# Alfieriek/Python-Temporal-AME-SVI

Measured on AMD Instinct MI355X. Metric: dyad-timestep ELBO updates/sec at n=1024,T=128,d=16; 1/2/4/8-GPU scaling, higher is better.
Workload: dtype f32

## Files before the change

python-temporal-ame-svi_amd/ame_amd/csrc/ame_sweep3.hip:

```cpp
#include "ame_common.h"
#include "ame_wave.h"
#include "ame_sweep_dev.h"

using namespace ame;

namespace {
__device__ __forceinline__ Mat2 inv2s_fast(Mat2 m) {
    const double det = m.a * m.d - m.b * m.c;
    double r = __builtin_amdgcn_rcp(det);
    r = fma(r, fma(-det, r, 1.0), r);
    r = fma(r, fma(-det, r, 1.0), r);
    const double o = 0.5 * (-m.b * r - m.c * r);
    return {m.d * r, o, o, m.a * r};
}
}

#ifdef AME_STAMPS
#define S3_I0 256
__device__ unsigned long long g_s3_stamps[8 * 16 * 16];
__device__ unsigned long long g_s3_prog[256 * 5];
__device__ unsigned int g_s3_hwid[8];
#define S3W(w) (w)
#define STAMP3(slot)                                                                           \
    do {                                                                                       \
// ... 101 lines not shown
    const int n = dm.n, TL = dm.T_local, Tt = dm.T_total;
    const int b = blockIdx.x;
    const int tl = (TL % 8 == 0) ? ((b & 7) * (TL >> 3) + (b >> 3)) : b;
    const int tg = dm.t_begin + tl;
    const int tid = threadIdx.x, lane = tid & 63, wave = __builtin_amdgcn_readfirstlane(tid >> 6);
    const int hl = tid - 64, hw = wave - 1;
    const int hj = (hl + kNH - kGOFF) % kNH;
    constexpr bool is_naive = VAR == AME_NAIVE, is_bad = VAR == AME_BAD;
    const int ns = (n + kNH - 1) / kNH;
    const int NY = (n * 8 + 1023) / 1024;
    const int KDMA = NY + NC + 2;

    extern __shared__ __attribute__((aligned(16))) char smem[];
    using LY = Lay<R>;
    const int YS = LY::ys(n);
    double* Kbuf = (double*)(smem + LY::oK);
    constexpr int KS = LY::KS, KSZ = LY::KSZ;
    constexpr int MCP = LY::MCP;
    double* arQ = (double*)(smem + LY::oAR);
    double* arP = arQ + D * MCP;
    double* rec = (double*)(smem + LY::oRec);
    double* mu64 = (double*)(smem + LY::oMu64);
    float* mu32 = (float*)(smem + LY::oMu32);
    double* g64 = (double*)(smem + LY::oG);
    double* jn64 = (double*)(smem + LY::oJn);
    double* vbuf = (double*)(smem + LY::oV);
    double* red = (double*)(smem + LY::oRed);
    float* gp = (float*)(smem + LY::oGP);
    float* yst = (float*)(smem + LY::oYst);
    float* muL = (float*)(smem + LY::oMuL);
    double* pdl = (double*)(smem + LY::oPd);
    double* pcdl = (double*)(smem + LY::oPc);
    double* ssq = (double*)(smem + LY::oSq);
    uint32_t* flags = (uint32_t*)(smem + LY::oFlag);
    uint32_t* kcnt = flags;
    uint32_t* gcnt = flags + 2;
    float2* yring = (float2*)(smem + LY::oYr);
    float* cring = (float*)(smem + LY::oCr);
    float* xring = (float*)(smem + LY::oXr);
    float* rring = (float*)(smem + LY::oRr);
    uint64_t* pring = (uint64_t*)(smem + LY::oPr);
    float* cst = (float*)(smem + LY::oCs);
    float2* mlds = (float2*)(smem + LY::oML(n));

    const double r00 = a.rinv[0], r01 = a.rinv[1], r10 = a.rinv[2], r11 = a.rinv[3];
    const float r00f = (float)r00, r01f = (float)r01, r10f = (float)r10, r11f = (float)r11;
    const Mat2 Rm = inv2s(m2(r00, r01, r10, r11));
    const float lr = a.lr, om = a.one_minus_lr;
    const float* xo = a.x_old + (size_t)tl * n * D;
    float* xn = a.x_new + (size_t)tl * n * D;
    float* cvs = a.cov + (size_t)tl * n * DD;
    float* cvw = (a.cov_new != nullptr ? a.cov_new : a.cov) + (size_t)tl * n * DD;
    const int nys = ame_ystride(n);
    const float* ysl = a.Yt + (size_t)tl * n * nys * 2;
    const bool back_rd = (a.wait_epoch != 0u) && (tl == TL - 1) && (a.back_in != nullptr);
    const float* xr = (tg < Tt - 1) ? ((tl < TL - 1) ? a.x_old + (size_t)(tl + 1) * n * D
                                                     : (back_rd ? a.back_in : a.next_old))
                                    : nullptr;
    const double* QiPhi = a.consts + 3 * (size_t)DD;
    bool dead = false;

    auto gran_src = [&](int node) -> const uint64_t* {
        return (tl == 0) ? a.halo_in + (size_t)node * D : a.hand + ((size_t)(tl - 1) * n + node) * D;
    };
    auto gran_finish = [&](int node, uint64_t v, float* dst) {
        if (tg == 0) {
            if (lane < D) dst[lane] = 0.f;
            return;
        }
        bool ok = (lane >= D) || (uint32_t)(v >> 32) == a.epoch;
        if (!__all(ok) && !dead) {
            const bool cross = tl == 0 && !(a.flags & AME_SWEEP_FLAG_PREV_GROUP);
            AmeSpin w(a.status, cross, lane == 0, hw == 0 ? AME_ST_HALO_US : 0);
            const uint64_t* src = gran_src(node);
            while (true) {
                bool stale = false;
                if (lane < D) {
                    v = cross ? gran_load_system(src + lane) : gran_load_agent(src + lane);
                    ok = (uint32_t)(v >> 32) == a.epoch;
                    stale = (uint32_t)(v >> 32) > a.epoch;
                }
                const bool st_hit = __any(stale);
                if (__all(ok) && !st_hit) break;
                const int r = st_hit ? 3 : w.poll();
                if (r != 0) {
                    const uint64_t bad = __ballot(!ok);
                    const int fl = bad ? (int)__builtin_ctzll(bad) : 0;
                    const uint32_t obs = (uint32_t)(__shfl(v, fl) >> 32);
                    if (lane == 0 && r >= 2)
                        ame_fail(a.status, (r == 3) ? AME_STATUS_STALE_EPOCH
                                                    : (cross ? AME_STATUS_HALO_TIMEOUT : AME_STATUS_SPIN_TIMEOUT),
                                 cross ? AME_WAIT_GRAN_HALO : AME_WAIT_GRAN_LOCAL, tg, (uint32_t)node, obs,
                                 a.epoch, w.waited(), a.epoch);
                    if (lane == 0)
                        __hip_atomic_fetch_or(gcnt, AME_LDS_DEAD, __ATOMIC_RELAXED, __HIP_MEMORY_SCOPE_WORKGROUP);
                    dead = true;
                    break;
                }
                __builtin_amdgcn_s_sleep(2);
            }
            w.end();
        }
        if (lane < D) dst[lane] = __uint_as_float((uint32_t)v);
    };

    auto dma_y = [&](int row) {
        const int rw = (row < n) ? row : 0;
        const char* base = (const char*)(ysl + (size_t)rw * nys * 2);
        const uint32_t dst = lds_off(yring + (size_t)(row & 3) * YS);
        for (int q = 0; q < NY; ++q) {
            int off = (q * 64 + lane) * 16;
            if (off >= n * 8) off = 0;
            dma16(base + off, dst + q * 1024);
        }
    };
    auto dma_cov = [&](int node) {
        const int cn = (node >= 0 && node < n) ? node : 0;
        const char* base = (const char*)(cvs + (size_t)cn * DD);
        const uint32_t dst = lds_off(cring + (size_t)(node & 3) * LY::cs);
#pragma unroll
        for (int q = 0; q < NC; ++q) {
            int off = (q * 64 + lane) * 16;
            if (off >= DD * 4) off = 0;
            dma16(base + off, dst + q * 1024);
        }
    };
    auto dma_x = [&](int node) {
        const int xnn = (node < n) ? node : 0;
        dma4(xo + (size_t)xnn * D + (lane < D ? lane : 0), lds_off(xring + (node & 7) * 64));
    };
    auto dma_r = [&](int node) {
        const float* src = (xr != nullptr && node < n) ? xr + (size_t)node * D : xo;
        if (back_rd) dma4_sys(src + (lane < D ? lane : 0), lds_off(rring + (node & 3) * 64));
        else dma4(src + (lane < D ? lane : 0), lds_off(rring + (node & 3) * 64));
    };

    auto flush_cov = [&](int node) {
        const float4* src = (const float4*)(cst + (size_t)((node + 1) & 1) * LY::cs);
        float4* dst = (float4*)(cvw + (size_t)node * DD);
#pragma unroll
        for (int q = 0; q < NC; ++q) {
            const int e = q * 64 + lane;
            if (e * 4 < DD) dst[e] = src[e];
        }
    };

#ifdef AME_STAMPS
    if (tl == TL / 2 && lane == 0) {
        unsigned int hwid;
        asm volatile("s_getreg_b32 %0, hwreg(HW_REG_HW_ID)" : "=s"(hwid));
        g_s3_hwid[wave] = hwid;
    }
#endif
    if (a.wait_epoch != 0u) {
        if (tid == 0) ame_wait_prev_done(a, tl, TL, tg, back_rd, n * D, dead);
        __syncthreads();
    }
    {
        double* piv = vbuf;
        double* K = Kbuf;
        const double pp = r00, ss = r11, qq = 0.5 * (r01 + r10);
        double* colsum = vbuf;
        float* x0 = (float*)(vbuf + M2);
        p0_gram_mfma<R, kNT / 64>(xo, n, D, K, KS, colsum, x0);
        if (tid < M2) {
            const int kq = 2 + (tid >= R ? tid - R : tid + R);
            const double v = (double)x0[tid];
            ssq[2 + tid] = fma(v, v, K[kq * KS + kq]);
        }
        __syncthreads();
        for (int e = tid; e < NLT; e += kNT) {
            int k, m;
            tri_decode3(e, k, m);
            double v;
            if (k < 2) {
                v = ((k == 0 && m == 0) ? pp : (k == 1 && m == 1) ? ss : qq) * (double)(n - 1);
            } else {
                const bool ku = (k - 2) < R;
                if (m < 2) {
                    const int ck = k - 2, kc = (ck < R) ? R + ck : ck - R;
                    v = (ku ? (m == 0 ? pp : qq) : (m == 0 ? qq : ss)) * colsum[kc];
                } else {
                    const bool mu_ = (m - 2) < R;
                    v = ((ku && mu_) ? pp : ((!ku && !mu_) ? ss : qq)) * K[k * KS + m];
                }
            }
            v += pconst_entry(a.consts, D, k, m, tg, Tt);
            K[k * KS + m] = v;
            K[m * KS + k] = v;
        }
        __syncthreads();
        for (int pv = 0; pv < D; ++pv) {
            if (tid < D) piv[tid] = K[pv * KS + tid];
            __syncthreads();
            const double rinv = 1.0 / piv[pv];
            for (int e = tid; e < NLT; e += kNT) {
                int k, m;
                tri_decode3(e, k, m);
                double v;
                if (k == pv && m == pv) v = -rinv;
                else if (k == pv) v = piv[m] * rinv;
                else if (m == pv) v = piv[k] * rinv;
                else v = K[k * KS + m] - (piv[k] * piv[m]) * rinv;
                K[k * KS + m] = v;
                K[m * KS + k] = v;
            }
            __syncthreads();
        }
        for (int e = tid; e < KSZ; e += kNT) K[e] = -K[e];
        __syncthreads();
    }
    for (int e = tid; e < 2 * D * MCP; e += kNT) {
        const int mat = e / (D * MCP), rc = e - mat * D * MCP, rr = rc / MCP, cc = rc - rr * MCP;
        arQ[e] = (cc < D) ? QiPhi[(size_t)mat * DD + rr * D + cc] : 0.0;
    }
    for (int e = tid; e < 3 * 64; e += kNT) muL[e] = 0.f;
    if (tid < D) pcdl[tid] = pconst_entry(a.consts, D, tid, tid, tg, Tt);
    constexpr int RS = LY::RS;
    for (int e = tid; e < 2 * D * RS; e += kNT) rec[e] = 0.0;
    for (int e = tid; e < 2 * D; e += kNT) {
        mu64[e] = 0.0;
        mu32[e] = 0.f;
    }
    if (tid < 16) yst[tid] = 0.f;
    if (tid < 4) flags[tid] = 0u;
    float mreg[NSREG][M2];
    if (wave >= 1) {
#pragma unroll
        for (int s = 0; s < NSREG; ++s) {
            const int j = hj + kNH * s;
            const bool ok = s < ns && j < n;
#pragma unroll
            for (int c = 0; c < M2; ++c) mreg[s][c] = ok ? xo[(size_t)j * D + 2 + c] : 0.f;
        }
        for (int s = NSREG; s < ns; ++s) {
            const int j = hj + kNH * s;
            const bool ok = j < n;
            for (int c2 = 0; c2 < MP; ++c2) {
                float2 v = make_float2(0.f, 0.f);
                if (ok) {
                    v.x = xo[(size_t)j * D + 2 + 2 * c2];
                    if (2 * c2 + 1 < M2) v.y = xo[(size_t)j * D + 3 + 2 * c2];
                }
                mlds[((s - NSREG) * MP + c2) * kNH + hl] = v;
            }
        }
        for (int e = hl; e < 2 * n; e += kNH) {
            const int rw = e / n, j = e - rw * n;
            yring[(size_t)rw * YS + j] = (rw < n) ? *(const float2*)(ysl + ((size_t)rw * nys + j) * 2)
                                                    : make_float2(0.f, 0.f);
        }
    }
    if (wave == 7) {
        for (int q = 0; q < 5; ++q) dma_x(q);
        for (int q = 0; q < 4; ++q) dma_r(q);
        asm volatile("s_waitcnt vmcnt(0)" ::: "memory");
    }
    __syncthreads();

    auto gemv = [&](int m, const float2* ysrc, int i) {
        float acc[D];
#pragma unroll
        for (int c = 0; c < D; ++c) acc[c] = 0.f;
        float2 yv[NSREG];
#pragma unroll
        for (int s = 0; s < NSREG; ++s) {
            const int j = hj + kNH * s;
            const float2 y = ysrc[j];
            yv[s] = (j < n) ? y : make_float2(0.f, 0.f);
        }
#pragma unroll
        for (int s = 0; s < NSREG; ++s) {
            if (s < ns) {
                const int j = hj + kNH * s;
                const bool ex = (j >= m - 2) && (j <= m);
                const float z0 = ex ? 0.f : r00f * yv[s].x + r01f * yv[s].y;
                const float z1 = ex ? 0.f : r10f * yv[s].x + r11f * yv[s].y;
                acc[0] += z0;
                acc[1] += z1;
#pragma unroll
                for (int c = 0; c < R; ++c) {
                    acc[2 + c] = fmaf(z0, mreg[s][R + c], acc[2 + c]);
                    acc[2 + R + c] = fmaf(z1, mreg[s][c], acc[2 + R + c]);
                }
            }
        }
        for (int s = NSREG; s < ns; ++s) {
            const int j = hj + kNH * s;
            float2 y = ysrc[j];
            if (j >= n) y = make_float2(0.f, 0.f);
            const bool ex = (j >= m - 2) && (j <= m);
            const float z0 = ex ? 0.f : r00f * y.x + r01f * y.y;
            const float z1 = ex ? 0.f : r10f * y.x + r11f * y.y;
            acc[0] += z0;
            acc[1] += z1;
            const float2* ml = mlds + (size_t)(s - NSREG) * MP * kNH + hl;
#pragma unroll
            for (int c2 = 0; c2 < MP; ++c2) {
                const float2 t = ml[c2 * kNH];
                const int c = 2 * c2;
                if (c < R) acc[2 + R + c] = fmaf(z1, t.x, acc[2 + R + c]);
                else acc[2 + (c - R)] = fmaf(z0, t.x, acc[2 + (c - R)]);
                if (c + 1 < M2) {
                    if (c + 1 < R) acc[2 + R + c + 1] = fmaf(z1, t.y, acc[2 + R + c + 1]);
                    else acc[2 + (c + 1 - R)] = fmaf(z0, t.y, acc[2 + (c + 1 - R)]);
                }
            }
        }
        STAMP3(7);
        int idx;
        const float v = wave_reduce_scatter<D>(acc, lane, idx);
        STAMP3(8);
        if (idx < D) gp[((m & 1) * 7 + hw) * D + idx] = v;
        const int jm1 = m - 1, jm2 = m - 2;
        if (jm1 >= 0 && ((jm1 + kGOFF) % kNH) == hl) {
            const float2 y = ysrc[jm1];
            yst[(m & 3) * 4 + 0] = y.x;
            yst[(m & 3) * 4 + 1] = y.y;
        }
        if (jm2 >= 0 && ((jm2 + kGOFF) % kNH) == hl) {
            const float2 y = ysrc[jm2];
            yst[(m & 3) * 4 + 2] = y.x;
            yst[(m & 3) * 4 + 3] = y.y;
        }
    };
    auto hf1 = [&](int m) {
        const int q = hl;
        const int k = q / NP, p = q - k * NP;
        const int kc = (k < D) ? k : 0;
        const float* ml = muL + hw * 64;
        const float* mr = rring + (m & 3) * 64;
        const double* aq = arQ + kc * MCP + p * MC;
        const double* ap = arP + kc * MCP + p * MC;
        double av[MC], bv[MC];
        float lv[MC], rv[MC], gv[7];
#pragma unroll
        for (int mm = 0; mm < MC; ++mm) {
            av[mm] = aq[mm];
            bv[mm] = ap[mm];
            lv[mm] = ml[p * MC + mm];
            rv[mm] = mr[p * MC + mm];
        }
#pragma unroll
        for (int w = 0; w < 7; ++w) gv[w] = gp[((m & 1) * 7 + w) * D + kc];
        const float mv2 = jcol_load<R>(mu32 + ((m - 2) & 1) * D, kc);
        const float ys0 = yst[(m & 3) * 4 + 2], ys1 = yst[(m & 3) * 4 + 3];
        __builtin_amdgcn_sched_barrier(0);
        double accL = 0.0, accR = 0.0;
#pragma unroll
        for (int mm = 0; mm < MC; ++mm) {
            accL = fma(av[mm], (double)lv[mm], accL);
            accR = fma(bv[mm], (double)rv[mm], accR);
        }
        double acc = accL + ((tg < Tt - 1) ? accR : 0.0);
        acc = dpp_add_xor1(acc);
        if constexpr (NP == 4) acc = dpp_add_mirror4(acc);
        double g = 0.0;
#pragma unroll
        for (int w = 0; w < 7; ++w) g += (double)gv[w];
        g += acc;
        if (m >= 2) {
            double j0, j1;
            jcol_sel<R>(mv2, true, kc, j0, j1);
            const double y0 = (double)ys0, y1 = (double)ys1;
            const double z0 = r00 * y0 + r01 * y1, z1 = r10 * y0 + r11 * y1;
            g = fma(j0, z0, fma(j1, z1, g));
        }
        if (k < D && p == 0) g64[(m & 1) * D + k] = g;
    };
    auto jn_fill = [&](int node) {
        if (lane < M2) {
            const float* xm = xring + (node & 7) * 64;
            jn64[(node & 1) * 2 * D + lane] = (node < n) ? (double)xm[2 + lane] : 0.0;
        }
    };

    if (wave >= 1) {
        gemv(0, yring, -1);
        gemv(1, yring + YS, -1);
        if (hw <= 2) {
            uint64_t g0 = 0;
            if (tg > 0 && lane < D)
                g0 = (tl == 0) ? gran_load_system(gran_src(0) + lane) : gran_load_agent(gran_src(0) + lane);
            gran_finish(0, g0, muL + hw * 64);
        }
        if (hw == 3) jn_fill(1);
    }
    __syncthreads();
    if (wave >= 1 && hw <= 2) hf1(0);
    __syncthreads();
    if (wave == 7) {
        for (int q = 2; q <= 4; ++q) dma_y(q);
        for (int q = 0; q <= 1; ++q) dma_cov(q);
        asm volatile("s_waitcnt vmcnt(0)" ::: "memory");
    }
    if (wave == 6 && lane < D) {
        uint64_t g1 = 0;
        if (tg > 0 && n > 1)
            g1 = (tl == 0) ? gran_load_system(gran_src(1) + lane) : gran_load_agent(gran_src(1) + lane);
        pring[(size_t)1 * 128 + lane] = g1;
    }
    __syncthreads();

    if (wave == 0) {
        __builtin_amdgcn_s_setprio(3);
        dead = __any(dead) || (*(volatile uint32_t*)gcnt & AME_LDS_DEAD) != 0u;
        const int k = lane;
        const bool kl = k < D;
        const int kc = kl ? k : 0;
        double brow[D];
#pragma unroll
        for (int c = 0; c < D; ++c) brow[c] = kl ? Kbuf[(size_t)k * KS + c] : 0.0;
        double v = 0, yv0 = 0, yv1 = 0, vA = 0, nq0 = 0, nq1 = 0;
        auto prep = [&](int node) {
            const double* jx = jn64 + ((node + 1) & 1) * 2 * D;
            if (!kl) return;
            const double* gg = g64 + (node & 1) * D;
            const bool ex1 = node + 1 < n;
            double s0 = 0, t0 = 0, s1 = ex1 ? brow[0] : 0.0, t1 = 0, s2 = ex1 ? brow[1] : 0.0, t2 = 0;
#pragma unroll
            for (int c = 0; c < D; c += 2) {
                s0 = fma(brow[c], gg[c], s0);
                t0 = fma(brow[c + 1], gg[c + 1], t0);
            }
#pragma unroll
            for (int c = 0; c < R; c += 2) {
                s1 = fma(brow[2 + c], jx[R + c], s1);
                s2 = fma(brow[2 + R + c], jx[c], s2);
                if (c + 1 < R) {
                    t1 = fma(brow[3 + c], jx[R + c + 1], t1);
                    t2 = fma(brow[3 + R + c], jx[c + 1], t2);
                }
            }
            v = s0 + t0;
            yv0 = s1 + t1;
            yv1 = s2 + t2;
            vA = brow[0] * gg[0] + brow[1] * gg[1];
            const double xj = jx[(k >= 2 && k < 2 + R) ? k - 2 + R : ((k >= 2 + R && k < D) ? k - 2 - R : 0)];
            nq0 = (k == 0) ? (ex1 ? 1.0 : 0.0) : ((k >= 2 && k < 2 + R) ? xj : 0.0);
            nq1 = (k == 1) ? (ex1 ? 1.0 : 0.0) : ((k >= 2 + R && k < D) ? xj : 0.0);
        };
        prep(0);
        double Wp0 = 0, Wp1 = 0, Xp0 = 0, Xp1 = 0, Lp0 = 0, Lp1 = 0, Gp0 = 0, Gp1 = 0;
        Mat2 Mip = m2(0, 0, 0, 0), Sip = m2(0, 0, 0, 0);
        for (int i = 0; i < n; ++i) {
            PROG3();
            STAMP3(0);
            const int par = i & 1, ppar = (i + 1) & 1;
            const bool has_prev = i > 0;
            const float* mup = mu32 + ppar * D;
            const double* mupd = mu64 + ppar * D;
            const double msk = kl ? 1.0 : 0.0;
            const double g = msk * g64[par * D + kc];
#if AME_S3_MOLD_EARLY
            const float mold_pf = xring[(i & 7) * 64 + kc];
#endif
            double J0, J1;
            jcol<R>(mup, has_prev && kl, kc, J0, J1);
            double kj0 = 0, kj1 = 0;
            if (has_prev) {
                double s0a = brow[0], s0b = 0, s1a = brow[1], s1b = 0;
#pragma unroll
                for (int c = 0; c < R; c += 2) {
                    s0a = fma(brow[2 + c], mupd[2 + R + c], s0a);
                    s1a = fma(brow[2 + R + c], mupd[2 + c], s1a);
                    if (c + 1 < R) {
                        s0b = fma(brow[3 + c], mupd[3 + R + c], s0b);
                        s1b = fma(brow[3 + R + c], mupd[3 + c], s1b);
                    }
                }
                kj0 = s0a + s0b;
                kj1 = s1a + s1b;
            }
            STAMP3(1);
            constexpr bool pack = is_naive;
            constexpr int NV = is_bad ? 40 : (pack ? 32 : 34);
            constexpr int IE = pack ? 11 : 12, IJY = IE + 2, INY = IJY + 4;
            constexpr int IB = INY + (pack ? 3 : 4), IF1 = IB + 4, IF2 = IF1 + 4;
            double pr[NV];
            pr[0] = Wp0 * J0; pr[1] = Wp0 * J1; pr[2] = Wp1 * J0; pr[3] = Wp1 * J1;
            pr[4] = Xp0 * J0; pr[5] = Xp0 * J1; pr[6] = Xp1 * J0; pr[7] = Xp1 * J1;
            if constexpr (!pack) {
                pr[8] = J0 * kj0; pr[9] = J0 * kj1; pr[10] = J1 * kj0; pr[11] = J1 * kj1;
            } else {
                pr[8] = J0 * kj0; pr[9] = 0.5 * (J0 * kj1 + J1 * kj0); pr[10] = J1 * kj1;
            }
            pr[IE] = J0 * v; pr[IE + 1] = J1 * v;
            pr[IJY] = J0 * yv0; pr[IJY + 1] = J0 * yv1; pr[IJY + 2] = J1 * yv0; pr[IJY + 3] = J1 * yv1;
            if constexpr (!pack) {
                pr[INY] = nq0 * yv0; pr[INY + 1] = nq0 * yv1; pr[INY + 2] = nq1 * yv0; pr[INY + 3] = nq1 * yv1;
            } else {
                pr[INY] = nq0 * yv0; pr[INY + 1] = 0.5 * (nq0 * yv1 + nq1 * yv0); pr[INY + 2] = nq1 * yv1;
            }
            pr[IB] = Wp0 * g; pr[IB + 1] = Wp1 * g; pr[IB + 2] = Xp0 * g; pr[IB + 3] = Xp1 * g;
            pr[IF1] = Wp0 * nq0; pr[IF1 + 1] = Wp0 * nq1; pr[IF1 + 2] = Wp1 * nq0; pr[IF1 + 3] = Wp1 * nq1;
            pr[IF2] = Xp0 * nq0; pr[IF2 + 1] = Xp0 * nq1; pr[IF2 + 2] = Xp1 * nq0; pr[IF2 + 3] = Xp1 * nq1;
            if constexpr (is_bad) {
                const double gA = (k < 2) ? g : 0.0;
                pr[34] = J0 * vA; pr[35] = J1 * vA;
                pr[36] = Wp0 * gA; pr[37] = Wp1 * gA; pr[38] = Xp0 * gA; pr[39] = Xp1 * gA;
            }
            {
                int idx;
                const double sv = wave_reduce_scatter<NV>(pr, lane, idx);
                if (idx < NV) red[idx] = sv;
            }
            wave_lds_sync3();
            double o[NV];
#pragma unroll
            for (int q = 0; q < NV; ++q) o[q] = red[q];
            const Mat2 a1 = m2(o[0], o[1], o[2], o[3]);
            const Mat2 a2 = m2(o[4], o[5], o[6], o[7]);
            const Mat2 cc = !pack ? m2(o[8], o[9], o[10], o[11]) : m2(o[8], o[9], o[9], o[10]);
            const V2 e = {o[IE], o[IE + 1]};
            const Mat2 jy = m2(o[IJY], o[IJY + 1], o[IJY + 2], o[IJY + 3]);
            const Mat2 ny = !pack ? m2(o[INY], o[INY + 1], o[INY + 2], o[INY + 3])
                                   : m2(o[INY], o[INY + 1], o[INY + 1], o[INY + 2]);
            STAMP3(2);
            STAMP3(3);
            const V2 b1 = {o[IB], o[IB + 1]}, b2 = {o[IB + 2], o[IB + 3]};
            const Mat2 f1 = m2(o[IF1], o[IF1 + 1], o[IF1 + 2], o[IF1 + 3]);
            const Mat2 f2 = m2(o[IF2], o[IF2 + 1], o[IF2 + 2], o[IF2 + 3]);
            double y0 = 0, y1 = 0;
            if (has_prev) { y0 = (double)yst[(i & 3) * 4 + 0]; y1 = (double)yst[(i & 3) * 4 + 1]; }
            const double zp0 = r00 * y0 + r01 * y1, zp1 = r10 * y0 + r11 * y1;
            const Mat2 JW = add(sub(cc, quad(a1, Mip, a1)), quad(a2, Sip, a2));
            const Mat2 Mm = add(Rm, sym(JW));
            const Mat2 Mi = has_prev ? inv2s_fast(Mm) : m2(0, 0, 0, 0);
            const V2 t1 = mtv(a1, mv(Mip, b1)), t2 = mtv(a2, mv(Sip, b2));
            const V2 Ju = {e.x - t1.x + t2.x, e.y - t1.y + t2.y};
            const V2 cvec = mv(Mi, V2{y0 - Ju.x, y1 - Ju.y});
            const Mat2 wn = add(sub(jy, quad(a1, Mip, f1)), quad(a2, Sip, f2));
            const Mat2 JnK = add(sub(ny, quad(f1, Mip, f1)), quad(f2, Sip, f2));
            const Mat2 JnX = sub(JnK, quad(wn, Mi, wn));
            const Mat2 Si = inv2s_fast(sub(Rm, sym(JnX)));
            const double W0 = kj0 - (Lp0 * a1.a + Lp1 * a1.c) + (Gp0 * a2.a + Gp1 * a2.c);
            const double W1 = kj1 - (Lp0 * a1.b + Lp1 * a1.d) + (Gp0 * a2.b + Gp1 * a2.d);
            const double u = v - (Lp0 * b1.x + Lp1 * b1.y) + (Gp0 * b2.x + Gp1 * b2.y);
            const double kn0 = yv0 - (Lp0 * f1.a + Lp1 * f1.c) + (Gp0 * f2.a + Gp1 * f2.c);
            const double kn1 = yv1 - (Lp0 * f1.b + Lp1 * f1.d) + (Gp0 * f2.b + Gp1 * f2.d);
            double mus;
            if constexpr (!is_bad) {
                mus = u + W0 * cvec.x + W1 * cvec.y;
            } else {
                const V2 eA = {o[34], o[35]};
                const V2 b1A = {o[36], o[37]}, b2A = {o[38], o[39]};
                const double uA = vA - (Lp0 * b1A.x + Lp1 * b1A.y) + (Gp0 * b2A.x + Gp1 * b2A.y);
// ... 319 lines not shown
```

python-temporal-ame-svi_amd/ame_amd/csrc/ame_sweep_dev.h:

```cpp
#pragma once
#include "ame_common.h"
#include "ame_wave.h"

namespace ame {

__device__ __forceinline__ void lds_barrier3() {
    asm volatile("s_waitcnt lgkmcnt(0)" ::: "memory");
    __builtin_amdgcn_s_barrier();
    asm volatile("" ::: "memory");
}
__device__ __forceinline__ void wave_lds_sync3() {
    asm volatile("s_waitcnt lgkmcnt(0)" ::: "memory");
    __builtin_amdgcn_wave_barrier();
    asm volatile("" ::: "memory");
}
__device__ __forceinline__ void lds_signal_add(uint32_t* f, uint32_t v) {
    asm volatile("s_waitcnt lgkmcnt(0)" ::: "memory");
    __hip_atomic_fetch_add(f, v, __ATOMIC_RELAXED, __HIP_MEMORY_SCOPE_WORKGROUP);
}
__device__ __forceinline__ void lds_signal_set(uint32_t* f, uint32_t v) {
    asm volatile("s_waitcnt lgkmcnt(0)" ::: "memory");
    __hip_atomic_store(f, v, __ATOMIC_RELAXED, __HIP_MEMORY_SCOPE_WORKGROUP);
}
#define AME_LDS_DEAD 0x40000000u
static __device__ __attribute__((noinline)) uint32_t lds_wait_slow(uint32_t* f, uint32_t target, uint32_t* status,
                                                                   int slice, uint32_t node, uint32_t epoch) {
    const bool ld = (threadIdx.x & 63) == 0;
    AmeSpin w(status, false, ld);
    uint32_t v;
    while ((v = __hip_atomic_load(f, __ATOMIC_RELAXED, __HIP_MEMORY_SCOPE_WORKGROUP)) < target) {
        __builtin_amdgcn_s_sleep(8);
        const int r = w.poll();
        if (r == 0) continue;
        if (r == 2 && ld)
            ame_fail(status, AME_STATUS_LDS_TIMEOUT, AME_WAIT_LDS, slice, node, v, target, w.waited(), epoch);
        v |= AME_LDS_DEAD;
        break;
    }
    w.end();
    return v;
}
__device__ __forceinline__ void lds_wait_ge(uint32_t* f, uint32_t target, uint32_t* status, bool& dead,
                                            int slice = 0, uint32_t node = AME_NODE_NONE,
                                            uint32_t epoch = 0) {
    uint32_t v = __hip_atomic_load(f, __ATOMIC_RELAXED, __HIP_MEMORY_SCOPE_WORKGROUP);
    if (!dead && v < target) v = lds_wait_slow(f, target, status, slice, node, epoch);
    dead = dead || (v & AME_LDS_DEAD) != 0u;
    asm volatile("" ::: "memory");
}

__device__ __forceinline__ void ame_wait_prev_done(const ame_sweep_args& a, int t, int TL, int tg,
                                                   bool back_rd, int nd, bool& dead, bool account = true) {
    const int qn = (t + 1 < TL || (a.flags & AME_SWEEP_FLAG_NEXT_GROUP)) ? 2 : 1;
    for (int q = 0; q <= qn && !dead; ++q) {
        const bool back = q == qn;
        if (back && !back_rd) break;
        const uint32_t* w = back ? (const uint32_t*)(a.back_in + AME_BACK_DONE_OFFSET(nd)) : a.done + t + q;
        const int site = back ? AME_WAIT_BACK : (q == 0 ? AME_WAIT_DONE_SELF : AME_WAIT_DONE_RIGHT);
        auto load = [&]() -> uint32_t {
            return back ? __hip_atomic_load(const_cast<uint32_t*>(w), __ATOMIC_RELAXED, __HIP_MEMORY_SCOPE_SYSTEM)
                        : __hip_atomic_load(const_cast<uint32_t*>(w), __ATOMIC_RELAXED, __HIP_MEMORY_SCOPE_AGENT);
        };
        uint32_t dv = load();
        if (dv == a.wait_epoch) continue;
        AmeSpin sp(a.status, back, true, (back && account) ? AME_ST_BACK_US : 0);
        while (true) {
            if (dv > a.wait_epoch) {
                ame_fail(a.status, AME_STATUS_STALE_EPOCH, site, tg, AME_NODE_NONE, dv, a.wait_epoch,
                         sp.waited(), a.epoch);
                dead = true;
                break;
            }
            if (dv == a.wait_epoch) break;
            const int r = sp.poll();
            if (r != 0) {
                if (r == 2)
                    ame_fail(a.status, back ? AME_STATUS_HALO_TIMEOUT : AME_STATUS_SPIN_TIMEOUT, site, tg,
                             AME_NODE_NONE, dv, a.wait_epoch, sp.waited(), a.epoch);
                dead = true;
                break;
            }
            __builtin_amdgcn_s_sleep(8);
            dv = load();
        }
        sp.end();
    }
    if (back_rd) __builtin_amdgcn_fence(__ATOMIC_ACQUIRE, "");
    __builtin_amdgcn_fence(__ATOMIC_ACQUIRE, "agent");
    asm volatile("s_waitcnt vmcnt(0)" ::: "memory");
}

typedef double ame_p0d4 __attribute__((ext_vector_type(4)));
template <int R, int NW>
__device__ __forceinline__ void p0_gram_mfma(const float* xo, int n, int D, double* gram, int ks,
                                             double* colsum, float* x0) {
    constexpr int M2 = 2 * R, NT = (M2 + 15) / 16, NTL = NT * (NT + 1) / 2;
    const int tid = threadIdx.x, lane = tid & 63, w = tid >> 6;
    const int ci = lane & 15, ck = lane >> 4;
    ame_p0d4 acc[NTL];
#pragma unroll
    for (int t = 0; t < NTL; ++t) acc[t] = ame_p0d4{0.0, 0.0, 0.0, 0.0};
    double cs[NT];
#pragma unroll
    for (int I = 0; I < NT; ++I) cs[I] = 0.0;
    const int nch = (n + 3) / 4;
    constexpr int U = 4;
    for (int c0 = w; c0 < nch; c0 += NW * U) {
        float xv[U][NT];
#pragma unroll
        for (int u = 0; u < U; ++u) {
            const int j = 4 * (c0 + NW * u) + ck;
#pragma unroll
            for (int I = 0; I < NT; ++I) {
                const int col = 16 * I + ci;
                const bool ok = j >= 1 && j < n && col < M2;
                xv[u][I] = ok ? xo[(size_t)j * D + 2 + col] : 0.f;
            }
        }
#pragma unroll
        for (int u = 0; u < U; ++u) {
            double xd[NT];
#pragma unroll
            for (int I = 0; I < NT; ++I) {
                xd[I] = (double)xv[u][I];
                cs[I] += xd[I];
            }
#pragma unroll
            for (int I = 0; I < NT; ++I)
#pragma unroll
                for (int J = 0; J <= I; ++J) {
                    const int t = I * (I + 1) / 2 + J;
                    acc[t] = __builtin_amdgcn_mfma_f64_16x16x4f64(xd[I], xd[J], acc[t], 0, 0, 0);
                }
        }
    }
#pragma unroll
    for (int I = 0; I < NT; ++I) {
        const double s1 = cs[I] + __shfl_xor(cs[I], 16);
        cs[I] = s1 + __shfl_xor(s1, 32);
    }
    auto kk = [](int a) { return 2 + (a >= R ? a - R : a + R); };
    for (int ww = 0; ww < NW; ++ww) {
        if (w == ww) {
#pragma unroll
            for (int I = 0; I < NT; ++I)
#pragma unroll
                for (int J = 0; J <= I; ++J) {
                    const int t = I * (I + 1) / 2 + J;
#pragma unroll
                    for (int v = 0; v < 4; ++v) {
                        const int a = 16 * I + ck + 4 * v, b = 16 * J + ci;
                        if (a >= M2 || b >= M2) continue;
                        double* p = gram + kk(a) * ks + kk(b);
                        double* q = gram + kk(b) * ks + kk(a);
                        const double g = acc[t][v];
                        *p = (ww == 0) ? g : *p + g;
                        if (I != J) *q = *p;
                    }
                }
            if (ck == 0) {
#pragma unroll
                for (int I = 0; I < NT; ++I) {
                    const int a = 16 * I + ci;
                    if (a < M2) colsum[a] = (ww == 0) ? cs[I] : colsum[a] + cs[I];
                }
            }
        }
        __syncthreads();
    }
    if (tid < M2) x0[tid] = xo[2 + tid];
    __syncthreads();
}

__device__ __forceinline__ uint32_t lds_off(const void* p) {
    return __builtin_amdgcn_readfirstlane((uint32_t)(uintptr_t)p);
}
__device__ __forceinline__ void dma16(const void* gsrc, uint32_t lds) {
    uint32_t keep;
    asm volatile("s_mov_b32 %0, m0\n\ts_mov_b32 m0, %2\n\ts_nop 0\n\tglobal_load_lds_dwordx4 %1, off\n\ts_mov_b32 m0, %0"
                 : "=&s"(keep) : "v"(gsrc), "s"(lds) : "memory");
}
__device__ __forceinline__ void dma16_sc1(const void* gsrc, uint32_t lds) {
    uint32_t keep;
    asm volatile("s_mov_b32 %0, m0\n\ts_mov_b32 m0, %2\n\ts_nop 0\n\tglobal_load_lds_dwordx4 %1, off sc1\n\ts_mov_b32 m0, %0"
                 : "=&s"(keep) : "v"(gsrc), "s"(lds) : "memory");
}
__device__ __forceinline__ void dma16_sys(const void* gsrc, uint32_t lds) {
    uint32_t keep;
    asm volatile("s_mov_b32 %0, m0\n\ts_mov_b32 m0, %2\n\ts_nop 0\n\tglobal_load_lds_dwordx4 %1, off sc0 sc1\n\ts_mov_b32 m0, %0"
                 : "=&s"(keep) : "v"(gsrc), "s"(lds) : "memory");
}
__device__ __forceinline__ void dma4_sys(const void* gsrc, uint32_t lds) {
    uint32_t keep;
    asm volatile("s_mov_b32 %0, m0\n\ts_mov_b32 m0, %2\n\ts_nop 0\n\tglobal_load_lds_dword %1, off sc0 sc1\n\ts_mov_b32 m0, %0"
                 : "=&s"(keep) : "v"(gsrc), "s"(lds) : "memory");
}
__device__ __forceinline__ void dma4(const void* gsrc, uint32_t lds) {
    uint32_t keep;
    asm volatile("s_mov_b32 %0, m0\n\ts_mov_b32 m0, %2\n\ts_nop 0\n\tglobal_load_lds_dword %1, off\n\ts_mov_b32 m0, %0"
                 : "=&s"(keep) : "v"(gsrc), "s"(lds) : "memory");
}
__device__ __forceinline__ void vm_wait_le(int n) {
    if (n >= 60) asm volatile("s_waitcnt vmcnt(60)" ::: "memory");
    else if (n >= 48) asm volatile("s_waitcnt vmcnt(48)" ::: "memory");
    else if (n >= 40) asm volatile("s_waitcnt vmcnt(40)" ::: "memory");
    else if (n >= 32) asm volatile("s_waitcnt vmcnt(32)" ::: "memory");
    else if (n >= 28) asm volatile("s_waitcnt vmcnt(28)" ::: "memory");
    else if (n >= 24) asm volatile("s_waitcnt vmcnt(24)" ::: "memory");
    else if (n >= 20) asm volatile("s_waitcnt vmcnt(20)" ::: "memory");
// ... 51 lines not shown
```

Measured before the change: 29.72 billion.

## Reorder sweep prologue to overlap setup and DMA with inter-block wait

Moves the LDS zero-fills, y-ring loads and early dma_y calls ahead of the previous-epoch wait, and splits that wait so only the self dependency blocks the Gram/inverse stage while the right-neighbour and back wait runs later on wave 7 before dma_r. The Gauss-Jordan inverse now ping-pongs between two Kbuf copies with precomputed triangle indices held in registers. This removes one barrier per pivot, folds the final negation into the last pivot, and drops a barrier before dma_y/dma_cov. The intent is to hide the cross-block wait and prologue latency. The cost is a second Kbuf copy in LDS, more registers, and more complex dead-flag propagation through gcnt.

New measurement: 29.82 billion, median of 5. About the same (+0.3%).

```diff
diff --git a/python-temporal-ame-svi_amd/ame_amd/csrc/ame_sweep3.hip b/python-temporal-ame-svi_amd/ame_amd/csrc/ame_sweep3.hip
--- a/python-temporal-ame-svi_amd/ame_amd/csrc/ame_sweep3.hip
+++ b/python-temporal-ame-svi_amd/ame_amd/csrc/ame_sweep3.hip
@@ -277,111 +277,263 @@
         g_s3_hwid[wave] = hwid;
     }
 #endif
-    if (a.wait_epoch != 0u) {
-        if (tid == 0) ame_wait_prev_done(a, tl, TL, tg, back_rd, n * D, dead);
+    constexpr bool kReordered = !is_naive;
+    constexpr int RS = LY::RS;
+    float mreg[NSREG][M2];
+    if constexpr (kReordered) {
+        auto early_fills = [&]() {
+        for (int e = tid; e < 2 * D * MCP; e += kNT) {
+            const int mat = e / (D * MCP), rc = e - mat * D * MCP, rr = rc / MCP, cc = rc - rr * MCP;
+            arQ[e] = (cc < D) ? QiPhi[(size_t)mat * DD + rr * D + cc] : 0.0;
+        }
+        for (int e = tid; e < 3 * 64; e += kNT) muL[e] = 0.f;
+        if (tid < D) pcdl[tid] = pconst_entry(a.consts, D, tid, tid, tg, Tt);
+        for (int e = tid; e < 2 * D * RS; e += kNT) rec[e] = 0.0;
+        for (int e = tid; e < 2 * D; e += kNT) {
+            mu64[e] = 0.0;
+            mu32[e] = 0.f;
+        }
+        if (tid < 16) yst[tid] = 0.f;
+        if (tid < 4) flags[tid] = 0u;
+        if (wave == 7) {
+            dma_y(2);
+            dma_y(3);
+        }
+        if (wave >= 1) {
+            for (int e = hl; e < 2 * n; e += kNH) {
+                const int rw = e / n, j = e - rw * n;
+                yring[(size_t)rw * YS + j] = (rw < n) ? *(const float2*)(ysl + ((size_t)rw * nys + j) * 2)
+                                                        : make_float2(0.f, 0.f);
+            }
+        }
+        };
+        early_fills();
+        constexpr int NQ = (NLT + kNT - 1) / kNT;
+        int pk_[NQ], pm_[NQ];
+#pragma unroll
+        for (int q = 0; q < NQ; ++q) {
+            const int e = tid + kNT * q;
+            int k = 0, m = 0;
+            if (e < NLT) tri_decode3(e, k, m);
+            pk_[q] = (e < NLT) ? k : -1;
+            pm_[q] = m;
+        }
+        if (a.wait_epoch != 0u) {
+            if (tid == 0) {
+                ame_wait_prev_done(a, tl, TL, tg, back_rd, n * D, dead, true, AME_WAIT_SEL_SELF);
+                if (dead) __hip_atomic_fetch_or(gcnt, AME_LDS_DEAD, __ATOMIC_RELAXED, __HIP_MEMORY_SCOPE_WORKGROUP);
+            }
+            __syncthreads();
+        }
+        if (wave == 7) {
+            for (int q = 0; q < 5; ++q) dma_x(q);
+            for (int q = 0; q <= 1; ++q) dma_cov(q);
+        }
+        {
+            double* K = Kbuf;
+            const double pp = r00, ss = r11, qq = 0.5 * (r01 + r10);
+            double* colsum = vbuf;
+            float* x0 = (float*)(vbuf + M2);
+            p0_gram_mfma<R, kNT / 64>(xo, n, D, K, KS, colsum, x0);
+            if (tid < M2) {
+                const int kq = 2 + (tid >= R ? tid - R : tid + R);
+                const double v = (double)x0[tid];
+                ssq[2 + tid] = fma(v, v, K[kq * KS + kq]);
+            }
+            __syncthreads();
+#pragma unroll
+            for (int q = 0; q < NQ; ++q) {
+                const int k = pk_[q], m = pm_[q];
+                if (k < 0) continue;
+                double v;
+                if (k < 2) {
+                    v = ((k == 0 && m == 0) ? pp : (k == 1 && m == 1) ? ss : qq) * (double)(n - 1);
+                } else {
+                    const bool ku = (k - 2) < R;
+                    if (m < 2) {
+                        const int ck = k - 2, kc = (ck < R) ? R + ck : ck - R;
+                        v = (ku ? (m == 0 ? pp : qq) : (m == 0 ? qq : ss)) * colsum[kc];
+                    } else {
+                        const bool mu_ = (m - 2) < R;
+                        v = ((ku && mu_) ? pp : ((!ku && !mu_) ? ss : qq)) * K[k * KS + m];
+                    }
+                }
+                v += pconst_entry(a.consts, D, k, m, tg, Tt);
+                K[k * KS + m] = v;
+                K[m * KS + k] = v;
+            }
+            __syncthreads();
+            auto load_node_rows = [&]() {
+            if (wave >= 1) {
+#pragma unroll
+                for (int s = 0; s < NSREG; ++s) {
+                    const int j = hj + kNH * s;
+                    const bool ok = s < ns && j < n;
+#pragma unroll
+                    for (int c = 0; c < M2; ++c) mreg[s][c] = ok ? xo[(size_t)j * D + 2 + c] : 0.f;
+                }
+            }
+            };
+            static_assert(D % 2 == 0, "the ping-pong inverse ends in Kbuf[0]");
+            for (int pv = 0; pv < D; ++pv) {
+                const double* Ks = Kbuf + (size_t)(pv & 1) * KSZ;
+                double* Kd = Kbuf + (size_t)((pv + 1) & 1) * KSZ;
+                const double* piv = Ks + pv * KS;
+                double pa[NQ], pb[NQ], pc[NQ];
+#pragma unroll
+                for (int q = 0; q < NQ; ++q) {
+                    const int k = pk_[q] < 0 ? 0 : pk_[q], m = pm_[q];
+                    pa[q] = piv[k];
+                    pb[q] = piv[m];
+                    pc[q] = Ks[k * KS + m];
+                }
+                const double rinv = 1.0 / piv[pv];
+                const bool last = pv == D - 1;
+#pragma unroll
+                for (int q = 0; q < NQ; ++q) {
+                    const int k = pk_[q], m = pm_[q];
+                    const double vg = pc[q] - (pa[q] * pb[q]) * rinv;
+                    const double vr = (k == pv ? pb[q] : pa[q]) * rinv;
+                    double v = (k == pv && m == pv) ? -rinv : ((k == pv || m == pv) ? vr : vg);
+                    if (last) v = -v;
+                    if (k >= 0) {
+                        Kd[k * KS + m] = v;
+                        Kd[m * KS + k] = v;
+                    }
+                }
+                lds_barrier3();
+            }
+            load_node_rows();
+        }
+        if (wave >= 1) {
+            for (int s = NSREG; s < ns; ++s) {
+                const int j = hj + kNH * s;
+                const bool ok = j < n;
+                for (int c2 = 0; c2 < MP; ++c2) {
+                    float2 v = make_float2(0.f, 0.f);
+                    if (ok) {
+                        v.x = xo[(size_t)j * D + 2 + 2 * c2];
+                        if (2 * c2 + 1 < M2) v.y = xo[(size_t)j * D + 3 + 2 * c2];
+                    }
+                    mlds[((s - NSREG) * MP + c2) * kNH + hl] = v;
+                }
+            }
+        }
+        if (wave == 7) {
+            if (a.wait_epoch != 0u && lane == 0 &&
+                !(__hip_atomic_load(gcnt, __ATOMIC_RELAXED, __HIP_MEMORY_SCOPE_WORKGROUP) & AME_LDS_DEAD)) {
+                ame_wait_prev_done(a, tl, TL, tg, back_rd, n * D, dead, true, AME_WAIT_SEL_RIGHT);
+                if (dead) __hip_atomic_fetch_or(gcnt, AME_LDS_DEAD, __ATOMIC_RELAXED, __HIP_MEMORY_SCOPE_WORKGROUP);
+            }
+            for (int q = 0; q < 4; ++q) dma_r(q);
+            asm volatile("s_waitcnt vmcnt(0)" ::: "memory");
+        }
         __syncthreads();
-    }
-    {
-        double* piv = vbuf;
-        double* K = Kbuf;
-        const double pp = r00, ss = r11, qq = 0.5 * (r01 + r10);
-        double* colsum = vbuf;
-        float* x0 = (float*)(vbuf + M2);
-        p0_gram_mfma<R, kNT / 64>(xo, n, D, K, KS, colsum, x0);
-        if (tid < M2) {
-            const int kq = 2 + (tid >= R ? tid - R : tid + R);
-            const double v = (double)x0[tid];
-            ssq[2 + tid] = fma(v, v, K[kq * KS + kq]);
-        }
-        __syncthreads();
-        for (int e = tid; e < NLT; e += kNT) {
-            int k, m;
-            tri_decode3(e, k, m);
-            double v;
-            if (k < 2) {
-                v = ((k == 0 && m == 0) ? pp : (k == 1 && m == 1) ? ss : qq) * (double)(n - 1);
-            } else {
-                const bool ku = (k - 2) < R;
-                if (m < 2) {
-                    const int ck = k - 2, kc = (ck < R) ? R + ck : ck - R;
-                    v = (ku ? (m == 0 ? pp : qq) : (m == 0 ? qq : ss)) * colsum[kc];
-                } else {
-                    const bool mu_ = (m - 2) < R;
-                    v = ((ku && mu_) ? pp : ((!ku && !mu_) ? ss : qq)) * K[k * KS + m];
-                }
-            }
-            v += pconst_entry(a.consts, D, k, m, tg, Tt);
-            K[k * KS + m] = v;
-            K[m * KS + k] = v;
-        }
-        __syncthreads();
-        for (int pv = 0; pv < D; ++pv) {
-            if (tid < D) piv[tid] = K[pv * KS + tid];
+    } else {
+        if (a.wait_epoch != 0u) {
+            if (tid == 0) ame_wait_prev_done(a, tl, TL, tg, back_rd, n * D, dead);
             __syncthreads();
-            const double rinv = 1.0 / piv[pv];
+        }
+        {
+            double* piv = vbuf;
+            double* K = Kbuf;
+            const double pp = r00, ss = r11, qq = 0.5 * (r01 + r10);
+            double* colsum = vbuf;
+            float* x0 = (float*)(vbuf + M2);
+            p0_gram_mfma<R, kNT / 64>(xo, n, D, K, KS, colsum, x0);
+            if (tid < M2) {
+                const int kq = 2 + (tid >= R ? tid - R : tid + R);
+                const double v = (double)x0[tid];
+                ssq[2 + tid] = fma(v, v, K[kq * KS + kq]);
+            }
+            __syncthreads();
             for (int e = tid; e < NLT; e += kNT) {
                 int k, m;
                 tri_decode3(e, k, m);
                 double v;
-                if (k == pv && m == pv) v = -rinv;
-                else if (k == pv) v = piv[m] * rinv;
-                else if (m == pv) v = piv[k] * rinv;
-                else v = K[k * KS + m] - (piv[k] * piv[m]) * rinv;
+                if (k < 2) {
+                    v = ((k == 0 && m == 0) ? pp : (k == 1 && m == 1) ? ss : qq) * (double)(n - 1);
+                } else {
+                    const bool ku = (k - 2) < R;
+                    if (m < 2) {
+                        const int ck = k - 2, kc = (ck < R) ? R + ck : ck - R;
+                        v = (ku ? (m == 0 ? pp : qq) : (m == 0 ? qq : ss)) * colsum[kc];
+                    } else {
+                        const bool mu_ = (m - 2) < R;
+                        v = ((ku && mu_) ? pp : ((!ku && !mu_) ? ss : qq)) * K[k * KS + m];
+                    }
+                }
+                v += pconst_entry(a.consts, D, k, m, tg, Tt);
                 K[k * KS + m] = v;
                 K[m * KS + k] = v;
             }
             __syncthreads();
-        }
-        for (int e = tid; e < KSZ; e += kNT) K[e] = -K[e];
+            for (int pv = 0; pv < D; ++pv) {
+                if (tid < D) piv[tid] = K[pv * KS + tid];
+                __syncthreads();
+                const double rinv = 1.0 / piv[pv];
+                for (int e = tid; e < NLT; e += kNT) {
+                    int k, m;
+                    tri_decode3(e, k, m);
+                    double v;
+                    if (k == pv && m == pv) v = -rinv;
+                    else if (k == pv) v = piv[m] * rinv;
+                    else if (m == pv) v = piv[k] * rinv;
+                    else v = K[k * KS + m] - (piv[k] * piv[m]) * rinv;
+                    K[k * KS + m] = v;
+                    K[m * KS + k] = v;
+                }
+                __syncthreads();
+            }
+            for (int e = tid; e < KSZ; e += kNT) K[e] = -K[e];
+            __syncthreads();
+        }
+        for (int e = tid; e < 2 * D * MCP; e += kNT) {
+            const int mat = e / (D * MCP), rc = e - mat * D * MCP, rr = rc / MCP, cc = rc - rr * MCP;
+            arQ[e] = (cc < D) ? QiPhi[(size_t)mat * DD + rr * D + cc] : 0.0;
+        }
+        for (int e = tid; e < 3 * 64; e += kNT) muL[e] = 0.f;
+        if (tid < D) pcdl[tid] = pconst_entry(a.consts, D, tid, tid, tg, Tt);
+        for (int e = tid; e < 2 * D * RS; e += kNT) rec[e] = 0.0;
+        for (int e = tid; e < 2 * D; e += kNT) {
+            mu64[e] = 0.0;
+            mu32[e] = 0.f;
+        }
+        if (tid < 16) yst[tid] = 0.f;
+        if (tid < 4) flags[tid] = 0u;
+        if (wave >= 1) {
+#pragma unroll
+            for (int s = 0; s < NSREG; ++s) {
+                const int j = hj + kNH * s;
+                const bool ok = s < ns && j < n;
+#pragma unroll
+                for (int c = 0; c < M2; ++c) mreg[s][c] = ok ? xo[(size_t)j * D + 2 + c] : 0.f;
+            }
+            for (int s = NSREG; s < ns; ++s) {
+                const int j = hj + kNH * s;
+                const bool ok = j < n;
+                for (int c2 = 0; c2 < MP; ++c2) {
+                    float2 v = make_float2(0.f, 0.f);
+                    if (ok) {
+                        v.x = xo[(size_t)j * D + 2 + 2 * c2];
+                        if (2 * c2 + 1 < M2) v.y = xo[(size_t)j * D + 3 + 2 * c2];
+                    }
+                    mlds[((s - NSREG) * MP + c2) * kNH + hl] = v;
+                }
+            }
+            for (int e = hl; e < 2 * n; e += kNH) {
+                const int rw = e / n, j = e - rw * n;
+                yring[(size_t)rw * YS + j] = (rw < n) ? *(const float2*)(ysl + ((size_t)rw * nys + j) * 2)
+                                                        : make_float2(0.f, 0.f);
+            }
+        }
+        if (wave == 7) {
+            for (int q = 0; q < 5; ++q) dma_x(q);
+            for (int q = 0; q < 4; ++q) dma_r(q);
+            asm volatile("s_waitcnt vmcnt(0)" ::: "memory");
+        }
         __syncthreads();
     }
-    for (int e = tid; e < 2 * D * MCP; e += kNT) {
-        const int mat = e / (D * MCP), rc = e - mat * D * MCP, rr = rc / MCP, cc = rc - rr * MCP;
-        arQ[e] = (cc < D) ? QiPhi[(size_t)mat * DD + rr * D + cc] : 0.0;
-    }
-    for (int e = tid; e < 3 * 64; e += kNT) muL[e] = 0.f;
-    if (tid < D) pcdl[tid] = pconst_entry(a.consts, D, tid, tid, tg, Tt);
-    constexpr int RS = LY::RS;
-    for (int e = tid; e < 2 * D * RS; e += kNT) rec[e] = 0.0;
-    for (int e = tid; e < 2 * D; e += kNT) {
-        mu64[e] = 0.0;
-        mu32[e] = 0.f;
-    }
-    if (tid < 16) yst[tid] = 0.f;
-    if (tid < 4) flags[tid] = 0u;
-    float mreg[NSREG][M2];
-    if (wave >= 1) {
-#pragma unroll
-        for (int s = 0; s < NSREG; ++s) {
-            const int j = hj + kNH * s;
-            const bool ok = s < ns && j < n;
-#pragma unroll
-            for (int c = 0; c < M2; ++c) mreg[s][c] = ok ? xo[(size_t)j * D + 2 + c] : 0.f;
-        }
-        for (int s = NSREG; s < ns; ++s) {
-            const int j = hj + kNH * s;
-            const bool ok = j < n;
-            for (int c2 = 0; c2 < MP; ++c2) {
-                float2 v = make_float2(0.f, 0.f);
-                if (ok) {
-                    v.x = xo[(size_t)j * D + 2 + 2 * c2];
-                    if (2 * c2 + 1 < M2) v.y = xo[(size_t)j * D + 3 + 2 * c2];
-                }
-                mlds[((s - NSREG) * MP + c2) * kNH + hl] = v;
-            }
-        }
-        for (int e = hl; e < 2 * n; e += kNH) {
-            const int rw = e / n, j = e - rw * n;
-            yring[(size_t)rw * YS + j] = (rw < n) ? *(const float2*)(ysl + ((size_t)rw * nys + j) * 2)
-                                                    : make_float2(0.f, 0.f);
-        }
-    }
-    if (wave == 7) {
-        for (int q = 0; q < 5; ++q) dma_x(q);
-        for (int q = 0; q < 4; ++q) dma_r(q);
-        asm volatile("s_waitcnt vmcnt(0)" ::: "memory");
-    }
-    __syncthreads();
 
     auto gemv = [&](int m, const float2* ysrc, int i) {
         float acc[D];
@@ -513,11 +665,18 @@
     }
     __syncthreads();
     if (wave >= 1 && hw <= 2) hf1(0);
-    __syncthreads();
-    if (wave == 7) {
-        for (int q = 2; q <= 4; ++q) dma_y(q);
-        for (int q = 0; q <= 1; ++q) dma_cov(q);
-        asm volatile("s_waitcnt vmcnt(0)" ::: "memory");
+    if constexpr (kReordered) {
+        if (wave == 7) {
+            dma_y(4);
+            asm volatile("s_waitcnt vmcnt(0)" ::: "memory");
+        }
+    } else {
+        __syncthreads();
+        if (wave == 7) {
+            for (int q = 2; q <= 4; ++q) dma_y(q);
+            for (int q = 0; q <= 1; ++q) dma_cov(q);
+            asm volatile("s_waitcnt vmcnt(0)" ::: "memory");
+        }
     }
     if (wave == 6 && lane < D) {
         uint64_t g1 = 0;
diff --git a/python-temporal-ame-svi_amd/ame_amd/csrc/ame_sweep_dev.h b/python-temporal-ame-svi_amd/ame_amd/csrc/ame_sweep_dev.h
--- a/python-temporal-ame-svi_amd/ame_amd/csrc/ame_sweep_dev.h
+++ b/python-temporal-ame-svi_amd/ame_amd/csrc/ame_sweep_dev.h
@@ -49,12 +49,17 @@
     asm volatile("" ::: "memory");
 }
 
+#define AME_WAIT_SEL_SELF 1
+#define AME_WAIT_SEL_RIGHT 2
 __device__ __forceinline__ void ame_wait_prev_done(const ame_sweep_args& a, int t, int TL, int tg,
-                                                   bool back_rd, int nd, bool& dead, bool account = true) {
+                                                   bool back_rd, int nd, bool& dead, bool account = true,
+                                                   int which = AME_WAIT_SEL_SELF | AME_WAIT_SEL_RIGHT) {
     const int qn = (t + 1 < TL || (a.flags & AME_SWEEP_FLAG_NEXT_GROUP)) ? 2 : 1;
+    if (!(which & AME_WAIT_SEL_RIGHT)) back_rd = false;
     for (int q = 0; q <= qn && !dead; ++q) {
         const bool back = q == qn;
         if (back && !back_rd) break;
+        if (!(which & (q == 0 ? AME_WAIT_SEL_SELF : AME_WAIT_SEL_RIGHT))) continue;
         const uint32_t* w = back ? (const uint32_t*)(a.back_in + AME_BACK_DONE_OFFSET(nd)) : a.done + t + q;
         const int site = back ? AME_WAIT_BACK : (q == 0 ? AME_WAIT_DONE_SELF : AME_WAIT_DONE_RIGHT);
         auto load = [&]() -> uint32_t {
```
